# TheJacksonLaboratory/cnn_autoencoder

Hardware: AMD Instinct MI355X
Metric: tiles/sec, compress+decompress round trip of 1024x1024x3 histology tiles (higher is better)
Workload: dtype f32 (f16x3 split MFMA: 3 f16 MFMAs per product, fp32 accumulate)

## Files before the change

cnn_autoencoder_amd/csrc/cae_api.hip:

```cpp
#include "cae_hip.h"
#include "cae_internal.hpp"
#include "cae_kernels.hpp"
#include "cae_kernels_f16.hpp"
#include "cae_launch.hpp"
#include "cae_pack.hpp"

#include <algorithm>
#include <cmath>
#include <cstdio>
#include <cstdlib>
#include <cstring>
#include <string>

namespace cae {

thread_local std::string g_last_error;
thread_local int64_t g_last_ticket = 0;
thread_local int g_force_fp32 = 0;

int fail(int code, const char *fmt, ...) {
    char buf[512];
    va_list ap;
    va_start(ap, fmt);
    vsnprintf(buf, sizeof buf, fmt, ap);
    va_end(ap);
    g_last_error = buf;
    return code;
}

void dev_free(void *p) { (void)hipFree(p); }

int DevBuf::alloc(size_t n) {
    reset();
    HIP_TRY(hipMalloc(&p, n));
    bytes = n;
    return CAE_OK;
}

int DevBuf::upload(const void *src, size_t n) {
    CAE_TRY(alloc(n));
    HIP_TRY(hipMemcpy(p, src, n, hipMemcpyHostToDevice));
    return CAE_OK;
}

int Model::ensure_ws(int which, size_t bytes) {
    DevBuf &b = ws[which];
    if (b.bytes >= bytes) return CAE_OK;
    if (b) {
        HIP_TRY(hipDeviceSynchronize());
        b.reset();
    }
    return b.alloc((bytes + (1u << 20)) & ~(size_t)((1u << 20) - 1));
}

int Model::order_stream(void *stream) {
    if (last_stream_set && last_stream != stream) {
        if (!order_event) HIP_TRY(hipEventCreateWithFlags((hipEvent_t *)&order_event, hipEventDisableTiming));
        HIP_TRY(hipEventRecord((hipEvent_t)order_event, (hipStream_t)last_stream));
        HIP_TRY(hipStreamWaitEvent((hipStream_t)stream, (hipEvent_t)order_event, 0));
    }
    last_stream = stream;
    last_stream_set = true;
    return CAE_OK;
}

int Model::ensure_device() {
    if (!zero) {
        CAE_TRY(zero.alloc(1024));
        HIP_TRY(hipMemset(zero.p, 0, 1024));
    }
    if (medians_dirty && ent.channels > 0) {
        CAE_TRY(medians_dev.upload(ent.medians));
        medians_dirty = false;
    }
    if (density_dirty && !density.empty()) {
        CAE_TRY(density_dev.upload(density));
        density_dirty = false;
    }
    if (!flags) {
        HIP_TRY(hipHostMalloc((void **)&flags, kFlagSlots * sizeof(int), hipHostMallocMapped));
        memset(flags, 0, kFlagSlots * sizeof(int));
        HIP_TRY(hipHostGetDevicePointer((void **)&flags_dev, flags, 0));
    }
    return CAE_OK;
}

int *Model::next_flag(int64_t *ticket) {
    *ticket = ++flag_seq;
    const int slot = (int)(*ticket % kFlagSlots);
    *(volatile int *)(flags + slot) = 0;
    g_last_ticket = *ticket;
    return flags_dev + slot;
}

bool Model::f16_usable() const {
    if (precision != 1 || g_force_fp32) return false;
    for (auto *tr : {&enc, &dec})
        for (auto &l : *tr)
            if (l.set && l.f16_bad) return false;
    return true;
}

Model::~Model() {
    if (order_event) (void)hipEventDestroy((hipEvent_t)order_event);
    if (flags) (void)hipHostFree(flags);
}

struct ProfScope {
    Model *m;
    int track;
    hipStream_t st;
    std::vector<std::pair<void *, void *>> ev;
    hipEvent_t cur = nullptr;
    ProfScope(Model *m_, int track_, hipStream_t st_) : m(m_), track(track_), st(st_) {}
    void begin() {
        if (!m->profiling) return;
        hipEvent_t a;
        if (hipEventCreate(&a) != hipSuccess) return;
        (void)hipEventRecord(a, st);
        cur = a;
    }
    void end() {
        if (!m->profiling || !cur) return;
        hipEvent_t b;
        if (hipEventCreate(&b) != hipSuccess) return;
        (void)hipEventRecord(b, st);
        ev.emplace_back((void *)cur, (void *)b);
        cur = nullptr;
    }
    ~ProfScope() {
        if (m->profiling && !ev.empty()) m->prof[track].push_back(std::move(ev));
    }
};

static unsigned ew_grid(size_t total) {
    size_t b = (total + 255) / 256;
    return (unsigned)std::min<size_t>(std::max<size_t>(b, 1), 256 * 8 * 4);
}

static int layer_of(Model *m, int track, int index, Layer *&l) {
    if (track != CAE_ANALYSIS && track != CAE_SYNTHESIS) return fail(CAE_ERR_ARG, "bad track %d", track);
    if (index < 0 || index >= m->L) return fail(CAE_ERR_ARG, "layer index %d out of range", index);
    l = &(track == CAE_ANALYSIS ? m->enc : m->dec)[index];
    return CAE_OK;
}

static int upload_channels(DevBuf &d, const float *v, int c, int ct, float fill) {
    if (!v) {
        d.reset();
        return CAE_OK;
    }
    CAE_TRY(d.upload(pad_channels(v, c, ct, fill)));
    if ((uintptr_t)d.p % 16 != 0 || d.bytes != (size_t)ct * 32 * sizeof(float))
        return fail(CAE_ERR_HIP, "per-channel vector: device buffer %p (%zu bytes) is not a 16-byte aligned run of %d floats",
                    d.p, d.bytes, ct * 32);
    return CAE_OK;
}

static LayerArgs layer_args(const Model *m, const float *in, int in_planes, void *out, int n, int h, int w, int oh, int ow,
                            int ct, int cout, int outfmt, int act, int *flag) {
    LayerArgs a{};
    a.in = in;
    a.out = out;
    a.zero = m->zero.get<float>();
    a.medians = m->zero.get<float>();
    a.flag = flag;
    a.N = n;
    a.H = h;
    a.W = w;
    a.OH = oh;
    a.OW = ow;
    a.in_planes = in_planes;
    a.out_planes = ct * 4;
    a.cout = cout;
    a.outfmt = outfmt;
    a.act = act;
    return a;
}

}

using namespace cae;

template <int R>
static void launch_likelihood(Model *m, const float *y, int n, int hw, float *yhat, float *lik, double *part,
                              hipStream_t st) {
    hipLaunchKernelGGL(likelihood_kernel<R>, dim3(m->c_bn, n), dim3(256), 0, st, y, m->medians_dev.get<float>(),
                       m->density_dev.get<float>(), m->density_per_channel, m->density_k, m->density_bound,
                       m->likelihood_plain, m->c_bn, hw, yhat, lik, part);
}

static int set_stage(Model *m, int track, Layer &l, int stage, const float *w, const float *bias, const float *beta,
                     const float *gamma, int act, int add_residual, int post_act) {
    const int ctin = round_ct(l.cin);
    if (ctin < 0) return fail(CAE_ERR_UNSUPPORTED, "more than 192 channels not supported");
    if ((int)l.stages.size() <= stage) l.stages.resize(stage + 1);
    Layer::Stage &sg = l.stages[stage];
    const bool tr = track == CAE_SYNTHESIS;
    CAE_TRY(sg.wp.upload(pack_weights(w, tr, l.cin, l.cin, m->ks, ctin, tr)));
    CAE_TRY(upload_channels(sg.bias, bias, l.cin, ctin, 0.0f));
    sg.gdn = beta != nullptr;
    if (sg.gdn) {
        CAE_TRY(upload_channels(sg.beta, beta, l.cin, ctin, 1.0f));
        CAE_TRY(sg.gp.upload(pack_gamma(gamma, l.cin, ctin)));
    }
    sg.act = act;
    sg.add_res = add_residual != 0;
    sg.post_act = post_act;
    if (m->precision == 1) {
        if (!fits_f16(w, (size_t)l.cin * l.cin * m->ks * m->ks)) l.f16_bad = true;
        CAE_TRY(sg.wp16.upload(pack_weights_f16(w, tr, l.cin, l.cin, m->ks, ctin, tr)));
        if (sg.gdn) {
            if (!fits_f16(gamma, (size_t)l.cin * l.cin)) l.f16_bad = true;
            CAE_TRY(sg.gp16.upload(pack_gamma_f16(gamma, l.cin, ctin)));
        }
    }
    if (track == CAE_ANALYSIS) {
        l.wp_edge.reset();
        l.wp_edge16.reset();
    }
    return CAE_OK;
}

static int pick_slot(int a, int b) {
    for (int k = 1; k <= 3; ++k)
        if (k != a && k != b) return k;
    return 1;
}

static bool stages_need_fp32(const Layer &l) {
    if (round_ct(l.cin) <= 4) return false;
    for (const Layer::Stage &sg : l.stages)
        if (sg.gdn || sg.add_res || sg.post_act) return true;
    return false;
}

static int run_stages(Model *m, const Layer &l, bool synthesis, int n, int ch, int cw, const float *&cur, int &cur_idx,
                      int &cur_planes, hipStream_t st, bool f16 = false, int *flag = nullptr) {
    if (f16 && stages_need_fp32(l)) {
        const int tmp = pick_slot(cur_idx, cur_idx);
        const size_t rows = (size_t)n * cur_planes * ch;
        if (synthesis)
            hipLaunchKernelGGL(c8s_to_c8_kernel<true>, dim3(ew_grid(rows * cw)), dim3(256), 0, st, (const char *)cur,
                               (float *)m->ws[tmp].p, rows, cw);
        else
            hipLaunchKernelGGL(c8s_to_c8_kernel<false>, dim3(ew_grid(rows * cw)), dim3(256), 0, st, (const char *)cur,
                               (float *)m->ws[tmp].p, rows, cw);
        HIP_TRY(hipGetLastError());
        cur = (const float *)m->ws[tmp].p;
        cur_idx = tmp;
        int rc = run_stages(m, l, synthesis, n, ch, cw, cur, cur_idx, cur_planes, st, false, nullptr);
        if (rc) return rc;
        const int back = pick_slot(cur_idx, cur_idx);
        const size_t orows = (size_t)n * cur_planes * ch;
        if (synthesis)
            hipLaunchKernelGGL(c8_to_c8s_kernel<true>, dim3(ew_grid(orows * cw)), dim3(256), 0, st, cur, (char *)m->ws[back].p,
                               orows, cw, flag);
        else
            hipLaunchKernelGGL(c8_to_c8s_kernel<false>, dim3(ew_grid(orows * cw)), dim3(256), 0, st, cur, (char *)m->ws[back].p,
                               orows, cw, flag);
        HIP_TRY(hipGetLastError());
        cur = (const float *)m->ws[back].p;
        cur_idx = back;
        return CAE_OK;
    }
    const float *unit_in = cur;
    const int unit_idx = cur_idx, unit_planes = cur_planes;
    for (const Layer::Stage &sg : l.stages) {
        const int ctin = round_ct(l.cin);
        const int out_idx = pick_slot(unit_idx, cur_idx);
        LayerArgs b = layer_args(m, cur, cur_planes, m->ws[out_idx].p, n, ch, cw, ch, cw, ctin, l.cin, OUT_C8, sg.act,
                                 f16 ? flag : nullptr);
        b.bias = sg.bias.get<float>();
        b.beta = sg.beta.get<float>();
        b.res = sg.add_res ? unit_in : nullptr;
        b.res_planes = unit_planes;
        b.post_act = sg.post_act;
        int rc;
        if (f16) {
            if (!sg.wp16 || (sg.gdn && !sg.gp16)) return fail(CAE_ERR_ARG, "stage uploaded before precision 1 was selected");
            b.wp = sg.wp16.get<float>();
            b.gp = sg.gp16.get<float>();
            rc = launch_conv_s1_f16(m->ks, ctin, synthesis, sg.gdn, l.cin, b, st);
        } else {
            b.wp = sg.wp.get<float>();
            b.gp = sg.gp.get<float>();
            rc = launch_conv_s1(m->ks, ctin, synthesis, sg.gdn, l.cin, b, st);
        }
        if (rc) return rc;
        cur = (const float *)b.out;
        cur_idx = out_idx;
        cur_planes = ctin * 4;
    }
    return CAE_OK;
}

static int launch_color(Model *m, const Layer &l, bool f16, const float *in, int in_planes, int n, int h, int w, float *out,
                        int *flag, hipStream_t st) {
    const int ct = round_ct(l.color_cout);
    LayerArgs c = layer_args(m, in, in_planes, out, n, h, w, h, w, ct, l.color_cout, OUT_NCHW, 0, f16 ? flag : nullptr);
    c.bias = l.color_bias.get<float>();
    if (f16) {
        c.wp = l.color_wp16.get<float>();
        return launch_color_f16(m->ks, l.cout, c, st);
    }
    c.wp = l.color_wp.get<float>();
    return launch_conv_s1(m->ks, ct, false, false, l.cout, c, st);
}

extern "C" {

int cae_version(void) { return 1; }
const char *cae_last_error(void) { return g_last_error.c_str(); }
void cae_free(void *p) { free(p); }

int cae_model_create(int channels_org, int channels_net, int channels_bn, int compression_level, int kernel_size,
                     cae_model_t **out) {
    if (!out) return fail(CAE_ERR_ARG, "out is NULL");
    if (channels_org < 1 || channels_net < 1 || channels_bn < 1 || compression_level < 1)
        return fail(CAE_ERR_ARG, "bad model dimensions");
    if (kernel_size != 3 && kernel_size != 5)
        return fail(CAE_ERR_UNSUPPORTED, "kernel_size %d not supported (3 or 5)", kernel_size);
    Model *m = new Model();
    m->c_org = channels_org;
    m->c_net = channels_net;
    m->c_bn = channels_bn;
    m->L = compression_level;
    m->ks = kernel_size;
    m->enc.resize(m->L);
    m->dec.resize(m->L);
// ... 417 lines not shown
        for (int i = 0; i < nrun; ++i) {
            if (!m->dec[i].stages.empty())
                maxact = std::max(maxact, (size_t)n * round_ct(m->dec[i].cin) * 4 * ch * row_bytes(cw));
            ch *= 2;
            cw *= 2;
            if (i + 1 < m->L) maxact = std::max(maxact, (size_t)n * m->dec[i].ct * 4 * ch * row_bytes(cw));
        }
    }
    bool need_third_slot = false;
    for (int i = 0; i < nrun; ++i)
        need_third_slot |= m->dec[i].stages.size() > 1 || (f16 && stages_need_fp32(m->dec[i]));
    if (scale > 0 && !m->dec[stop].color_w4 && fmt == CAE_FMT_U8_HWC) {
        maxact = std::max(maxact, (size_t)n * m->dec[stop].color_cout * (lh << nrun) * (lw << nrun) * sizeof(float));
    }
    if ((rc = m->ensure_ws(0, in_bytes))) return rc;
    if (maxact && ((rc = m->ensure_ws(1, maxact)) || (rc = m->ensure_ws(2, maxact)))) return rc;
    if (maxact && need_third_slot && (rc = m->ensure_ws(3, maxact))) return rc;

    ProfScope prof(m, CAE_SYNTHESIS, st);
    prof.begin();
    const size_t tot = (size_t)n * p0 * lh * lw;
    if (f16)
        hipLaunchKernelGGL(nchw_to_c8s_kernel<true>, dim3(ew_grid(tot)), dim3(256), 0, st, latents, (char *)m->ws[0].p, n,
                           m->c_bn, lh, lw, p0, flag, symbols, m->medians_dev.get<float>());
    else
        hipLaunchKernelGGL(nchw_to_c8_kernel, dim3(ew_grid(tot)), dim3(256), 0, st, latents, (float *)m->ws[0].p, n,
                           m->c_bn, lh * lw, p0, symbols, m->medians_dev.get<float>());
    HIP_TRY(hipGetLastError());
    prof.end();

    bool use_pmap = false;
    if (f16 && scale == 0 && m->L >= 2 && m->ks == 3 && getenv("CAE_NO_PMAP") == nullptr) {
        const Layer &lp = m->dec[m->L - 2], &ll = m->dec[m->L - 1];
        use_pmap = ll.wp_pmap16 && !ll.gdn && ll.stages.empty() && lp.stages.empty() && lp.ct <= 4 && lp.cout == ll.cin &&
                   !(bridges && bridges[m->L - 2]) && !(colors && colors[m->L - 2]);
    }
    if (use_pmap) maxact = std::max(maxact, (size_t)n * (lh << (m->L - 1)) * (lw << (m->L - 1)) * 128);
    if (use_pmap && ((rc = m->ensure_ws(1, maxact)) || (rc = m->ensure_ws(2, maxact)))) return rc;

    const float *cur = (const float *)m->ws[0].p;
    int cur_planes = p0, ch = lh, cw = lw;
    int cur_idx = 0;
    for (int i = 0; i < nrun; ++i) {
        const Layer &l = m->dec[i];
        const bool last = i == m->L - 1;
        if (use_pmap && last) {
            prof.begin();
            const int gtx = (cw + 15) / 16, gty = (ch + 15) / 16;
            hipLaunchKernelGGL(pmap_gather_kernel, dim3((unsigned)((size_t)n * gtx * gty)), dim3(256), 0, st, cur,
                               l.bias.get<float>(), out, n, ch, cw, l.cout, fmt == CAE_FMT_U8_HWC ? OUT_U8HWC : OUT_NCHW, gtx,
                               gty);
            HIP_TRY(hipGetLastError());
            prof.end();
            break;
        }
        if (!l.stages.empty() && (rc = run_stages(m, l, true, n, ch, cw, cur, cur_idx, cur_planes, st, f16, flag))) return rc;
        const int out_idx = pick_slot(cur_idx, cur_idx);
        LayerArgs a = layer_args(m, cur, cur_planes, last ? out : m->ws[out_idx].p, n, ch, cw, 2 * ch, 2 * cw, l.ct, l.cout,
                                 last ? (fmt == CAE_FMT_U8_HWC ? OUT_U8HWC : OUT_NCHW) : OUT_C8, l.act, flag);
        a.wp = l.wp.get<float>();
        a.bias = l.bias.get<float>();
        a.gp = l.gp.get<float>();
        a.beta = l.beta.get<float>();
        if (use_pmap && i == m->L - 2) {
            a.outfmt = OUT_PMAP;
            a.pm = m->dec[m->L - 1].wp_pmap16.p;
        }
        prof.begin();
        if (f16) {
            a.gp = l.gp16.get<float>();
            if (last && l.wp_edge16 && last_f16_fits(m->ks, l.cin)) {
                a.wp = l.wp_edge16.get<float>();
                if ((rc = launch_last_f16(m->ks, l.cin, a, st))) return rc;
            } else {
                if (l.act && l.ct > 4)
                    return fail(CAE_ERR_UNSUPPORTED, "f16x3: LeakyReLU / ReLU synthesis layers wider than 128 channels run "
                                                     "on the fp32 path: set precision 0");
                a.wp = l.wp16.get<float>();
                if ((rc = launch_deconv_f16(m->ks, l.ct, l.gdn, l.cin, a, st))) return rc;
            }
        } else if (last && l.wp_edge) {
            a.wp = l.wp_edge.get<float>();
            if ((rc = launch_last(m->ks, l.cin, a, st))) return rc;
        } else {
            if ((rc = launch_deconv(m->ks, l.ct, l.gdn, l.cin, a, st))) return rc;
        }
        prof.end();
        if (!last && colors && colors[i]) {
            if (!l.color_wp) return fail(CAE_ERR_ARG, "colour layer %d not set", i);
            if (f16 && !l.color_wp16)
                return fail(CAE_ERR_UNSUPPORTED, "f16x3: colour layers to more than 32 channels run on the fp32 path: set precision 0");
            if ((rc = launch_color(m, l, f16, (const float *)a.out, l.ct * 4, n, a.OH, a.OW, colors[i], flag, st))) return rc;
        }
        if (!last && bridges && bridges[i]) {
            const size_t t2 = (size_t)n * l.cout * a.OH * a.OW;
            if (f16)
                hipLaunchKernelGGL(c8s_to_nchw_kernel<true>, dim3(ew_grid(t2)), dim3(256), 0, st, (const char *)a.out,
                                   bridges[i], n, l.cout, a.OH, a.OW, l.ct * 4);
            else
                hipLaunchKernelGGL(c8_to_nchw_kernel, dim3(ew_grid(t2)), dim3(256), 0, st, (const float *)a.out,
                                   bridges[i], n, l.cout, a.OH * a.OW, l.ct * 4);
            HIP_TRY(hipGetLastError());
        }
        cur = (const float *)a.out;
        cur_planes = l.ct * 4;
        ch = a.OH;
        cw = a.OW;
        cur_idx = out_idx;
    }
    if (scale > 0) {
        const Layer &l = m->dec[stop];
        const int ofmt = fmt == CAE_FMT_U8_HWC ? OUT_U8HWC : OUT_NCHW;
        prof.begin();
        if (l.color_w4) {
            if ((rc = launch_color_small(m->ks, f16, cur, cur_planes, l.cout, l.color_w4.get<float>(),
                                         l.color_bias.get<float>(), n, ch, cw, l.color_cout, out, ofmt, flag, st)))
                return rc;
        } else {
            float *img = ofmt == OUT_NCHW ? (float *)out : (float *)m->ws[pick_slot(cur_idx, cur_idx)].p;
            if ((rc = launch_color(m, l, f16, cur, cur_planes, n, ch, cw, img, flag, st))) return rc;
            if (ofmt == OUT_U8HWC && (rc = launch_nchw_to_u8hwc(img, out, n, l.color_cout, (size_t)ch * cw, st))) return rc;
        }
        prof.end();
    }
    return CAE_OK;
}

int cae_gdn_forward(cae_model_t *mm, int track, int index, const float *x, int n, int h, int w, float *y, void *stream) {
    Model *m = reinterpret_cast<Model *>(mm);
    if (!m || !x || !y) return fail(CAE_ERR_ARG, "NULL argument");
    Layer *lp;
    CAE_TRY(layer_of(m, track, index, lp));
    if (n < 1 || h < 1 || w < 1) return fail(CAE_ERR_ARG, "bad tensor shape");
    hipStream_t st = (hipStream_t)stream;
    std::lock_guard<std::mutex> lk(m->mu);
    const Layer &l = *lp;
    if (!l.set || !l.gdn) return fail(CAE_ERR_ARG, "layer has no GDN");
    const int planes = l.ct * 4;
    int rc;
    if ((rc = m->ensure_device()) || (rc = m->order_stream(stream))) return rc;
    if ((rc = m->ensure_ws(0, (size_t)n * planes * h * w * 32))) return rc;
    const size_t tot = (size_t)n * planes * h * w;
    hipLaunchKernelGGL(nchw_to_c8_kernel, dim3(ew_grid(tot)), dim3(256), 0, st, x, (float *)m->ws[0].p, n, l.cout, h * w,
                       planes);
    HIP_TRY(hipGetLastError());
    LayerArgs a = layer_args(m, (const float *)m->ws[0].p, planes, y, n, h, w, h, w, l.ct, l.cout, OUT_NCHW, 0, nullptr);
    a.gp = l.gp.get<float>();
    a.beta = l.beta.get<float>();
    return launch_gdn(l.ct, track == CAE_SYNTHESIS, a, st);
}

int cae_tile_sse(const uint8_t *a, const uint8_t *b, int n, size_t elems, double *sse, void *stream) {
    if (!a || !b || !sse) return fail(CAE_ERR_ARG, "NULL argument");
    if (n < 1 || n > 65535 || elems < 1) return fail(CAE_ERR_ARG, "bad shape");
    hipStream_t st = (hipStream_t)stream;
    unsigned long long *acc = reinterpret_cast<unsigned long long *>(sse);
    HIP_TRY(hipMemsetAsync(acc, 0, (size_t)n * 8, st));
    const unsigned bx = (unsigned)std::min<size_t>(std::max<size_t>(elems / 16 / 256, 1), 64);
    hipLaunchKernelGGL(tile_sse_kernel, dim3(bx, n), dim3(256), 0, st, a, b, elems, acc);
    HIP_TRY(hipGetLastError());
    hipLaunchKernelGGL(u64_to_f64_kernel, dim3((n + 255) / 256), dim3(256), 0, st, acc, sse, n);
    HIP_TRY(hipGetLastError());
    return CAE_OK;
}

int cae_tile_ssim(const uint8_t *a, const uint8_t *b, int n, int h, int w, int c, double *ssim, double *workspace,
                  size_t workspace_elems, void *stream) {
    if (!a || !b || !ssim || !workspace) return fail(CAE_ERR_ARG, "NULL argument");
    if (n < 1 || n > 65535 || c < 1) return fail(CAE_ERR_ARG, "bad shape");
    if (h < 7 || w < 7) return fail(CAE_ERR_ARG, "tiles must be at least 7x7 (the SSIM window)");
    const int oh = h - 6, ow = w - 6;
    const int bxr = (ow + 31) / 32, bpt = bxr * ((oh + 31) / 32);
    if (workspace_elems < (size_t)n * bpt)
        return fail(CAE_ERR_ARG, "workspace too small: %zu doubles needed", (size_t)n * bpt);
    hipStream_t st = (hipStream_t)stream;
    hipLaunchKernelGGL(tile_ssim_kernel, dim3(bpt, n), dim3(256), 0, st, a, b, h, w, c, bxr, bpt, workspace);
    HIP_TRY(hipGetLastError());
    hipLaunchKernelGGL(ssim_reduce_kernel, dim3(n), dim3(256), 0, st, workspace, bpt, (double)oh * ow * c, ssim);
    HIP_TRY(hipGetLastError());
    return CAE_OK;
}

int cae_tile_delta_e(const uint8_t *a, const uint8_t *b, int n, size_t pixels, double *delta, double *workspace,
                     size_t workspace_elems, void *stream) {
    if (!a || !b || !delta || !workspace) return fail(CAE_ERR_ARG, "NULL argument");
    if (n < 1 || n > 65535 || pixels < 1) return fail(CAE_ERR_ARG, "bad shape");
    const int bpt = (int)std::min<size_t>((pixels + 255) / 256, 128);
    if (workspace_elems < (size_t)n * bpt)
        return fail(CAE_ERR_ARG, "workspace too small: %zu doubles needed", (size_t)n * bpt);
    hipStream_t st = (hipStream_t)stream;
    hipLaunchKernelGGL(tile_delta_e_kernel, dim3(bpt, n), dim3(256), 0, st, a, b, pixels, bpt, workspace);
    HIP_TRY(hipGetLastError());
    hipLaunchKernelGGL(ssim_reduce_kernel, dim3(n), dim3(256), 0, st, workspace, bpt, (double)pixels, delta);
    HIP_TRY(hipGetLastError());
    return CAE_OK;
}

int cae_u8hwc_to_planes(const uint8_t *tiles, int n, int h, int w, int c, float *planes, void *stream) {
    if (!tiles || !planes) return fail(CAE_ERR_ARG, "NULL argument");
    if (n < 1 || h < 1 || w < 1 || c < 1) return fail(CAE_ERR_ARG, "bad shape");
    hipLaunchKernelGGL(u8hwc_to_planes_kernel, dim3(ew_grid((size_t)n * c * h * w)), dim3(256), 0, (hipStream_t)stream,
                       tiles, planes, n, h, w, c);
    HIP_TRY(hipGetLastError());
    return CAE_OK;
}

int cae_avgpool2(const float *in, int planes, int h, int w, float *out, void *stream) {
    if (!in || !out) return fail(CAE_ERR_ARG, "NULL argument");
    if (planes < 1 || h < 1 || w < 1) return fail(CAE_ERR_ARG, "bad shape");
    const int oh = (h + 2 * (h & 1) - 2) / 2 + 1, ow = (w + 2 * (w & 1) - 2) / 2 + 1;
    hipLaunchKernelGGL(avgpool2_kernel, dim3(ew_grid((size_t)planes * oh * ow)), dim3(256), 0, (hipStream_t)stream, in,
                       out, planes, h, w, oh, ow);
    HIP_TRY(hipGetLastError());
    return CAE_OK;
}

int cae_msssim_level(const float *x, const float *y, int planes, int h, int w, const float *window11, double *ssim_cs,
                     double *workspace, size_t workspace_elems, void *stream) {
    if (!x || !y || !window11 || !ssim_cs || !workspace) return fail(CAE_ERR_ARG, "NULL argument");
    if (planes < 1 || planes > 65535) return fail(CAE_ERR_ARG, "bad plane count");
    if (h < 11 || w < 11) return fail(CAE_ERR_ARG, "image smaller than the 11-tap window");
    const int oh = h - 10, ow = w - 10;
    const int bxr = (ow + 31) / 32, bpp = bxr * ((oh + 31) / 32);
    if (workspace_elems < (size_t)planes * bpp * 2)
        return fail(CAE_ERR_ARG, "workspace too small: %zu doubles needed", (size_t)planes * bpp * 2);
    hipStream_t st = (hipStream_t)stream;
    hipLaunchKernelGGL(msssim_level_kernel, dim3(bpp, planes), dim3(256), 0, st, x, y, h, w, bxr, bpp, window11, workspace);
    HIP_TRY(hipGetLastError());
    hipLaunchKernelGGL(msssim_reduce_kernel, dim3(planes), dim3(256), 0, st, workspace, bpp, (double)oh * ow, ssim_cs);
    HIP_TRY(hipGetLastError());
    return CAE_OK;
}

int cae_model_set_profiling(cae_model_t *mm, int enable) {
    Model *m = reinterpret_cast<Model *>(mm);
    if (!m) return fail(CAE_ERR_ARG, "NULL model");
    std::lock_guard<std::mutex> lk(m->mu);
    m->profiling = enable != 0;
    return CAE_OK;
}

int cae_model_get_profile(cae_model_t *mm, int track, double *ms, int n_slots, int *calls, int reset) {
    Model *m = reinterpret_cast<Model *>(mm);
    if (!m || !ms || n_slots < 1) return fail(CAE_ERR_ARG, "NULL argument");
    if (track != CAE_ANALYSIS && track != CAE_SYNTHESIS) return fail(CAE_ERR_ARG, "bad track %d", track);
    std::lock_guard<std::mutex> lk(m->mu);
    for (int i = 0; i < n_slots; ++i) ms[i] = 0.0;
    auto &calls_v = m->prof[track];
    for (auto &call : calls_v)
        for (size_t i = 0; i < call.size(); ++i) {
            HIP_TRY(hipEventSynchronize((hipEvent_t)call[i].second));
            float t = 0.f;
            HIP_TRY(hipEventElapsedTime(&t, (hipEvent_t)call[i].first, (hipEvent_t)call[i].second));
            if ((int)i < n_slots) ms[i] += t;
        }
    if (calls) *calls = (int)calls_v.size();
    if (reset) {
        for (auto &call : calls_v)
            for (auto &e : call) {
                (void)hipEventDestroy((hipEvent_t)e.first);
                (void)hipEventDestroy((hipEvent_t)e.second);
            }
        calls_v.clear();
    }
    return CAE_OK;
}

int cae_quantize(cae_model_t *mm, const float *latents, int n, int hw, int32_t *symbols, void *stream) {
    Model *m = reinterpret_cast<Model *>(mm);
    if (!m || !latents || !symbols) return fail(CAE_ERR_ARG, "NULL argument");
    if (m->ent.channels == 0) return fail(CAE_ERR_ARG, "entropy model not set");
    if (n < 1 || hw < 1) return fail(CAE_ERR_ARG, "bad shape");
    {
        std::lock_guard<std::mutex> lk(m->mu);
        int rc = m->ensure_device();
        if (rc) return rc;
    }
    const size_t total = (size_t)n * m->c_bn * hw;
    hipLaunchKernelGGL(quantize_kernel, dim3(ew_grid(total)), dim3(256), 0, (hipStream_t)stream, latents,
                       m->medians_dev.get<float>(), symbols, m->c_bn, hw, total);
    HIP_TRY(hipGetLastError());
    return CAE_OK;
}

int cae_model_set_density(cae_model_t *mm, int channels, int n_filters, const int *filters, const float *const *matrices,
                          const float *const *biases, const float *const *factors, float likelihood_bound) {
    Model *m = reinterpret_cast<Model *>(mm);
    if (!m || !filters || !matrices || !biases || !factors) return fail(CAE_ERR_ARG, "NULL argument");
    if (channels != m->c_bn) return fail(CAE_ERR_ARG, "density model has %d channels, model %d", channels, m->c_bn);
    if (n_filters < 1) return fail(CAE_ERR_UNSUPPORTED, "density network needs at least one hidden layer");
    int R = 0;
    for (int i = 0; i < n_filters; ++i) {
        if (filters[i] < 1) return fail(CAE_ERR_ARG, "filters[%d]=%d", i, filters[i]);
        R = std::max(R, filters[i]);
    }
    if (R > 8) return fail(CAE_ERR_UNSUPPORTED, "density filters wider than 8 are not supported (got %d)", R);
    for (int i = 0; i <= n_filters; ++i)
        if (!matrices[i] || !biases[i] || (i < n_filters && !factors[i])) return fail(CAE_ERR_ARG, "NULL parameter %d", i);
    const int K = n_filters;
    const int per = 3 * R + (K - 1) * (R * R + 2 * R) + R + 1;
    std::vector<float> packed((size_t)channels * per, 0.f);
    auto width = [&](int i) { return i == 0 ? 1 : (i == K + 1 ? 1 : filters[i - 1]); };
    for (int c = 0; c < channels; ++c) {
        float *o = packed.data() + (size_t)c * per;
        for (int i = 0; i <= K; ++i) {
            const int fin = width(i), fout = width(i + 1);
            const float *M = matrices[i] + (size_t)c * fout * fin;
            const float *b = biases[i] + (size_t)c * fout;
            const float *t = i < K ? factors[i] + (size_t)c * fout : nullptr;
            if (i == 0) {
                for (int j = 0; j < fout; ++j) { o[j] = M[j]; o[R + j] = b[j]; o[2 * R + j] = t[j]; }
                o += 3 * R;
            } else if (i < K) {
                for (int j = 0; j < fout; ++j) {
// ... 118 lines not shown
```

cnn_autoencoder_amd/csrc/cae_kernels.hpp:

```cpp
#pragma once
#include <hip/hip_runtime.h>
#include <stdint.h>
#include <type_traits>
#include <utility>

namespace cae {

typedef float f32x16 __attribute__((ext_vector_type(16)));
typedef float f32x4 __attribute__((ext_vector_type(4)));

enum OutFmt { OUT_C8 = 0, OUT_NCHW = 1, OUT_U8HWC = 2, OUT_SYM = 3, OUT_PMAP = 4 };

struct LayerArgs {
    const float *in;
    void *out;
    const float *wp;
    const float *bias;
    const float *gp;
    const float *beta;
    const float *zero;
    int N, H, W, OH, OW;
    int in_planes;
    int cci;
    int out_planes;
// ... 735 lines not shown
    for (size_t i = (size_t)blockIdx.x * blockDim.x + threadIdx.x; i < total; i += (size_t)gridDim.x * blockDim.x) {
        const size_t pix = i % HW;
        const size_t np = i / HW;
        const int plane = (int)(np % planes);
        const size_t n = np / planes;
        f32x4 lo, hi;
#pragma unroll
        for (int k = 0; k < 4; ++k) {
            const int c0 = plane * 8 + k, c1 = c0 + 4;
            if (sym) {
                lo[k] = c0 < C ? (float)sym[(n * C + c0) * HW + pix] + medians[c0] : 0.0f;
                hi[k] = c1 < C ? (float)sym[(n * C + c1) * HW + pix] + medians[c1] : 0.0f;
            } else {
                lo[k] = c0 < C ? in[(n * C + c0) * HW + pix] : 0.0f;
                hi[k] = c1 < C ? in[(n * C + c1) * HW + pix] : 0.0f;
            }
        }
        float *dst = out + i * 8;
        *(f32x4 *)dst = lo;
        *(f32x4 *)(dst + 4) = hi;
    }
}

static __global__ void c8_to_nchw_kernel(const float *in, float *out, int N, int C, int HW, int planes) {
    const size_t total = (size_t)N * C * HW;
    for (size_t i = (size_t)blockIdx.x * blockDim.x + threadIdx.x; i < total; i += (size_t)gridDim.x * blockDim.x) {
        const size_t pix = i % HW;
        const size_t nc = i / HW;
        const int c = (int)(nc % C);
        const size_t n = nc / C;
        out[i] = in[((n * planes + (c >> 3)) * HW + pix) * 8 + (c & 7)];
    }
}

static __global__ void quantize_kernel(const float *y, const float *medians, int32_t *sym, int C, int HW, size_t total) {
    for (size_t i = (size_t)blockIdx.x * blockDim.x + threadIdx.x; i < total; i += (size_t)gridDim.x * blockDim.x) {
        const int c = (int)((i / HW) % C);
        sym[i] = round_sym(y[i] - medians[c]);
    }
}

static __global__ void __launch_bounds__(1024)
quantize_export4_kernel(const float *y, const float *medians, int32_t *sym, int C, int HW4, size_t total4) {
    typedef int i32x4 __attribute__((ext_vector_type(4)));
    const size_t stride = (size_t)gridDim.x * blockDim.x;
    for (size_t i0 = (size_t)blockIdx.x * blockDim.x + threadIdx.x; i0 < total4; i0 += 4 * stride) {
        f32x4 v[4];
#pragma unroll
        for (int k = 0; k < 4; ++k) {
            const size_t i = i0 + k * stride;
            if (i < total4) v[k] = ((const f32x4 *)y)[i];
        }
#pragma unroll
        for (int k = 0; k < 4; ++k) {
            const size_t i = i0 + k * stride;
            if (i < total4) {
                const float med = medians[(i / HW4) % C];
                i32x4 q;
#pragma unroll
                for (int e = 0; e < 4; ++e) q[e] = round_sym(v[k][e] - med);
                ((i32x4 *)sym)[i] = q;
            }
        }
    }
}

static __global__ void dequantize_kernel(const int32_t *sym, const float *medians, float *y, int C, int HW, size_t total) {
    for (size_t i = (size_t)blockIdx.x * blockDim.x + threadIdx.x; i < total; i += (size_t)gridDim.x * blockDim.x) {
        const int c = (int)((i / HW) % C);
        y[i] = (float)sym[i] + medians[c];
    }
}

template <int R>
__device__ __forceinline__ float logits_cumulative(const float *__restrict__ p, int K, float x) {
    float v[R];
#pragma unroll
    for (int j = 0; j < R; ++j) {
        v[j] = p[j] * x + p[R + j];
        v[j] += p[2 * R + j] * tanhf(v[j]);
    }
    p += 3 * R;
    for (int i = 1; i < K; ++i) {
        float u[R];
#pragma unroll
        for (int j = 0; j < R; ++j) {
            float acc = 0.f;
#pragma unroll
            for (int k = 0; k < R; ++k) acc += p[j * R + k] * v[k];
            acc += p[R * R + j];
            u[j] = acc + p[R * R + R + j] * tanhf(acc);
        }
#pragma unroll
        for (int j = 0; j < R; ++j) v[j] = u[j];
        p += R * R + 2 * R;
    }
    float acc = 0.f;
#pragma unroll
    for (int k = 0; k < R; ++k) acc += p[k] * v[k];
    return acc + p[R];
}

__device__ __forceinline__ float sigmoidf(float x) { return 1.f / (1.f + expf(-x)); }

template <int R>
__global__ void __launch_bounds__(256)
likelihood_kernel(const float *__restrict__ y, const float *__restrict__ medians, const float *__restrict__ params,
                  int per_channel, int K, float bound, int plain, int C, int HW, float *__restrict__ yhat,
                  float *__restrict__ lik, double *__restrict__ bits_part) {
    const int c = blockIdx.x, n = blockIdx.y;
    const float *pc = params + (size_t)c * per_channel;
    const float med = medians[c];
    const size_t base = ((size_t)n * C + c) * HW;
    double bits = 0.0;
    for (int i = threadIdx.x; i < HW; i += 256) {
        const float q = rintf(y[base + i] - med) + med;
        const float lo = logits_cumulative<R>(pc, K, q - 0.5f);
        const float up = logits_cumulative<R>(pc, K, q + 0.5f);
        const float t = lo + up;
        const float sgn = t > 0.f ? -1.f : (t < 0.f ? 1.f : 0.f);
        float pr = plain ? sigmoidf(up) - sigmoidf(lo) : fabsf(sigmoidf(sgn * up) - sigmoidf(sgn * lo));
        pr = fmaxf(pr, bound);
        if (yhat) yhat[base + i] = q;
        if (lik) lik[base + i] = pr;
        bits -= (double)log2f(pr);
    }
    if (!bits_part) return;
    __shared__ double red[256];
    red[threadIdx.x] = bits;
    __syncthreads();
#pragma unroll
    for (int s = 128; s > 0; s >>= 1) {
        if ((int)threadIdx.x < s) red[threadIdx.x] += red[threadIdx.x + s];
        __syncthreads();
    }
    if (threadIdx.x == 0) bits_part[(size_t)n * C + c] = red[0];
}

static __global__ void bits_reduce_kernel(const double *part, int C, double *bits) {
    __shared__ double red[256];
    const int n = blockIdx.x;
    double a = 0.0;
    for (int c = threadIdx.x; c < C; c += 256) a += part[(size_t)n * C + c];
    red[threadIdx.x] = a;
    __syncthreads();
#pragma unroll
    for (int s = 128; s > 0; s >>= 1) {
        if ((int)threadIdx.x < s) red[threadIdx.x] += red[threadIdx.x + s];
        __syncthreads();
    }
    if (threadIdx.x == 0) bits[n] = red[0];
}

static __global__ void tile_sse_kernel(const uint8_t *a, const uint8_t *b, size_t elems, unsigned long long *out) {
    const int tile = blockIdx.y;
    const uint8_t *pa = a + (size_t)tile * elems, *pb = b + (size_t)tile * elems;
    unsigned long long acc = 0;
    const bool vec = ((((uintptr_t)pa) | ((uintptr_t)pb)) & 15) == 0;
    const size_t nvec = vec ? elems / 16 : 0;
    auto sq = [](const uint4 &va, const uint4 &vb) {
        const unsigned wa[4] = {va.x, va.y, va.z, va.w}, wb[4] = {vb.x, vb.y, vb.z, vb.w};
        unsigned same = 0, cross = 0;
#pragma unroll
        for (int k = 0; k < 4; ++k) {
            same = __builtin_amdgcn_udot4(wa[k], wa[k], same, false);
            same = __builtin_amdgcn_udot4(wb[k], wb[k], same, false);
            cross = __builtin_amdgcn_udot4(wa[k], wb[k], cross, false);
        }
        return same - 2u * cross;
    };
    const size_t stride = (size_t)gridDim.x * blockDim.x;
    size_t i = (size_t)blockIdx.x * blockDim.x + threadIdx.x;
    for (; i + stride < nvec; i += 2 * stride) {
        const uint4 va0 = ((const uint4 *)pa)[i], vb0 = ((const uint4 *)pb)[i];
        const uint4 va1 = ((const uint4 *)pa)[i + stride], vb1 = ((const uint4 *)pb)[i + stride];
        acc += sq(va0, vb0);
        acc += sq(va1, vb1);
    }
    if (i < nvec) acc += sq(((const uint4 *)pa)[i], ((const uint4 *)pb)[i]);
    if (vec) {
        if (blockIdx.x == 0)
            for (size_t i = nvec * 16 + threadIdx.x; i < elems; i += blockDim.x) {
                const int d = (int)pa[i] - (int)pb[i];
                acc += (unsigned)(d * d);
            }
    } else {
        for (size_t i = (size_t)blockIdx.x * blockDim.x + threadIdx.x; i < elems; i += (size_t)gridDim.x * blockDim.x) {
            const int d = (int)pa[i] - (int)pb[i];
            acc += (unsigned)(d * d);
        }
    }
#pragma unroll
    for (int off = 32; off > 0; off >>= 1) acc += __shfl_down(acc, off, 64);
    if ((threadIdx.x & 63) == 0) atomicAdd(out + tile, acc);
}

static __global__ void __launch_bounds__(256)
tile_ssim_kernel(const uint8_t *a, const uint8_t *b, int H, int W, int C, int bx_per_row, int blocks_per_tile,
                 double *part) {
    constexpr int T = 32, WIN = 7, IN = T + WIN - 1;
    __shared__ uint8_t sa[IN][IN + 2], sb[IN][IN + 2];
    __shared__ int hs[5][IN][T];
    __shared__ double red[256];
    const int tile = blockIdx.y, blk = blockIdx.x;
    const int by = blk / bx_per_row, bx = blk - by * bx_per_row;
    const int oy0 = by * T, ox0 = bx * T;
    const int OH = H - WIN + 1, OW = W - WIN + 1;
    const size_t base = (size_t)tile * H * W * C;
    const double C1 = (0.01 * 255.0) * (0.01 * 255.0), C2 = (0.03 * 255.0) * (0.03 * 255.0);
    const double cov_norm = 49.0 / 48.0;
    double acc = 0.0;
    for (int c = 0; c < C; ++c) {
        __syncthreads();
        for (int i = threadIdx.x; i < IN * IN; i += 256) {
            const int r = i / IN, x = i - r * IN;
            const int iy = oy0 + r, ix = ox0 + x;
            const bool ok = iy < H && ix < W;
            const size_t off = base + ((size_t)(ok ? iy : 0) * W + (ok ? ix : 0)) * C + c;
            sa[r][x] = ok ? a[off] : 0;
            sb[r][x] = ok ? b[off] : 0;
        }
        __syncthreads();
        for (int i = threadIdx.x; i < IN * T; i += 256) {
            const int r = i / T, x = i - r * T;
            int s0 = 0, s1 = 0, s2 = 0, s3 = 0, s4 = 0;
#pragma unroll
            for (int k = 0; k < WIN; ++k) {
                const int u = sa[r][x + k], v = sb[r][x + k];
                s0 += u;
                s1 += v;
                s2 += u * u;
                s3 += v * v;
                s4 += u * v;
            }
            hs[0][r][x] = s0;
            hs[1][r][x] = s1;
            hs[2][r][x] = s2;
            hs[3][r][x] = s3;
            hs[4][r][x] = s4;
        }
        __syncthreads();
        for (int i = threadIdx.x; i < T * T; i += 256) {
            const int y = i / T, x = i - y * T;
            if (oy0 + y < OH && ox0 + x < OW) {
                int s[5] = {0, 0, 0, 0, 0};
#pragma unroll
                for (int k = 0; k < WIN; ++k)
#pragma unroll
                    for (int q = 0; q < 5; ++q) s[q] += hs[q][y + k][x];
                {
#pragma clang fp contract(off)
                    const double ux = s[0] / 49.0, uy = s[1] / 49.0;
                    const double vx = cov_norm * (s[2] / 49.0 - ux * ux), vy = cov_norm * (s[3] / 49.0 - uy * uy);
                    const double vxy = cov_norm * (s[4] / 49.0 - ux * uy);
                    const double A1 = 2.0 * ux * uy + C1, A2 = 2.0 * vxy + C2;
                    const double B1 = ux * ux + uy * uy + C1, B2 = vx + vy + C2;
                    acc += (A1 * A2) / (B1 * B2);
                }
            }
        }
    }
    red[threadIdx.x] = acc;
    __syncthreads();
#pragma unroll
    for (int st = 128; st > 0; st >>= 1) {
        if ((int)threadIdx.x < st) red[threadIdx.x] += red[threadIdx.x + st];
        __syncthreads();
    }
    if (threadIdx.x == 0) part[(size_t)tile * blocks_per_tile + blk] = red[0];
}

static __global__ void ssim_reduce_kernel(const double *part, int blocks_per_tile, double samples, double *ssim) {
    __shared__ double red[256];
    const int tile = blockIdx.x;
    double v = 0.0;
    for (int i = threadIdx.x; i < blocks_per_tile; i += 256) v += part[(size_t)tile * blocks_per_tile + i];
    red[threadIdx.x] = v;
    __syncthreads();
#pragma unroll
    for (int st = 128; st > 0; st >>= 1) {
        if ((int)threadIdx.x < st) red[threadIdx.x] += red[threadIdx.x + st];
        __syncthreads();
    }
    if (threadIdx.x == 0) ssim[tile] = red[0] / samples;
}

__device__ __forceinline__ void rgb_to_lab(const double *lin, const uint8_t *px, double &L, double &A, double &B) {
#pragma clang fp contract(off)
    const double r = lin[px[0]], g = lin[px[1]], b = lin[px[2]];
    double x = (0.412453 * r + 0.357580 * g + 0.180423 * b) / 0.95047;
    double y = (0.212671 * r + 0.715160 * g + 0.072169 * b) / 1.0;
    double z = (0.019334 * r + 0.119193 * g + 0.950227 * b) / 1.08883;
    x = x > 0.008856 ? cbrt(x) : 7.787 * x + 16.0 / 116.0;
    y = y > 0.008856 ? cbrt(y) : 7.787 * y + 16.0 / 116.0;
    z = z > 0.008856 ? cbrt(z) : 7.787 * z + 16.0 / 116.0;
    L = 116.0 * y - 16.0;
    A = 500.0 * (x - y);
    B = 200.0 * (y - z);
}

static __global__ void __launch_bounds__(256)
tile_delta_e_kernel(const uint8_t *a, const uint8_t *b, size_t pixels, int blocks_per_tile, double *part) {
    __shared__ double lin[256];
    __shared__ double red[256];
    {
        const double v = threadIdx.x / 255.0;
        lin[threadIdx.x] = v > 0.04045 ? pow((v + 0.055) / 1.055, 2.4) : v / 12.92;
    }
    __syncthreads();
    const int tile = blockIdx.y;
    const uint8_t *pa = a + (size_t)tile * pixels * 3, *pb = b + (size_t)tile * pixels * 3;
    double acc = 0.0;
    for (size_t i = (size_t)blockIdx.x * 256 + threadIdx.x; i < pixels; i += (size_t)blocks_per_tile * 256) {
#pragma clang fp contract(off)
        double l0, a0, b0, l1, a1, b1;
        rgb_to_lab(lin, pa + 3 * i, l0, a0, b0);
        rgb_to_lab(lin, pb + 3 * i, l1, a1, b1);
        acc += sqrt((l0 - l1) * (l0 - l1) + (a0 - a1) * (a0 - a1) + (b0 - b1) * (b0 - b1));
    }
    red[threadIdx.x] = acc;
    __syncthreads();
#pragma unroll
    for (int st = 128; st > 0; st >>= 1) {
        if ((int)threadIdx.x < st) red[threadIdx.x] += red[threadIdx.x + st];
        __syncthreads();
    }
    if (threadIdx.x == 0) part[(size_t)tile * blocks_per_tile + blockIdx.x] = red[0];
}

static __global__ void u8hwc_to_planes_kernel(const uint8_t *in, float *out, int N, int H, int W, int C) {
    const size_t total = (size_t)N * C * H * W;
    for (size_t i = (size_t)blockIdx.x * blockDim.x + threadIdx.x; i < total; i += (size_t)gridDim.x * blockDim.x) {
        const size_t pix = i % ((size_t)H * W);
        const size_t nc = i / ((size_t)H * W);
        const int c = (int)(nc % C);
        const size_t n = nc / C;
        out[i] = (float)in[(n * H * W + pix) * C + c];
    }
}

static __global__ void avgpool2_kernel(const float *in, float *out, int planes, int H, int W, int OH, int OW) {
    const int ph = H & 1, pw = W & 1;
    const size_t total = (size_t)planes * OH * OW;
    for (size_t i = (size_t)blockIdx.x * blockDim.x + threadIdx.x; i < total; i += (size_t)gridDim.x * blockDim.x) {
        const int ox = (int)(i % OW), oy = (int)((i / OW) % OH);
        const size_t pl = i / ((size_t)OW * OH);
        float s = 0.f;
#pragma unroll
        for (int dy = 0; dy < 2; ++dy)
#pragma unroll
            for (int dx = 0; dx < 2; ++dx) {
                const int y = 2 * oy - ph + dy, x = 2 * ox - pw + dx;
                if (y >= 0 && y < H && x >= 0 && x < W) s += in[(pl * H + y) * W + x];
            }
        out[i] = s * 0.25f;
    }
}

static __global__ void __launch_bounds__(256)
msssim_level_kernel(const float *X, const float *Y, int H, int W, int bx_per_row, int bpp, const float *win, double *part) {
    constexpr int T = 32, WIN = 11, IN = T + WIN - 1;
    __shared__ float sx[IN][IN + 1], sy[IN][IN + 1];
    __shared__ float vs[5][T][IN + 1];
    __shared__ double red[2][256];
    __shared__ float g[WIN];
    if (threadIdx.x < WIN) g[threadIdx.x] = win[threadIdx.x];
    const int plane = blockIdx.y, blk = blockIdx.x;
    const int by = blk / bx_per_row, bx = blk - by * bx_per_row;
    const int oy0 = by * T, ox0 = bx * T;
    const int OH = H - WIN + 1, OW = W - WIN + 1;
    const float *px = X + (size_t)plane * H * W, *py = Y + (size_t)plane * H * W;
    for (int i = threadIdx.x; i < IN * IN; i += 256) {
        const int r = i / IN, x = i - r * IN;
        const int iy = oy0 + r, ix = ox0 + x;
        const bool ok = iy < H && ix < W;
        sx[r][x] = ok ? px[(size_t)iy * W + ix] : 0.f;
        sy[r][x] = ok ? py[(size_t)iy * W + ix] : 0.f;
    }
    __syncthreads();
    for (int i = threadIdx.x; i < T * IN; i += 256) {
        const int y = i / IN, x = i - y * IN;
        float a0 = 0.f, a1 = 0.f, a2 = 0.f, a3 = 0.f, a4 = 0.f;
#pragma unroll
        for (int k = 0; k < WIN; ++k) {
            const float u = sx[y + k][x], v = sy[y + k][x], w = g[k];
            a0 = fmaf(w, u, a0);
            a1 = fmaf(w, v, a1);
            a2 = fmaf(w, u * u, a2);
            a3 = fmaf(w, v * v, a3);
            a4 = fmaf(w, u * v, a4);
        }
        vs[0][y][x] = a0;
        vs[1][y][x] = a1;
        vs[2][y][x] = a2;
        vs[3][y][x] = a3;
        vs[4][y][x] = a4;
    }
    __syncthreads();
    const float C1 = (0.01f * 255.f) * (0.01f * 255.f), C2 = (0.03f * 255.f) * (0.03f * 255.f);
    double ssum = 0.0, csum = 0.0;
    for (int i = threadIdx.x; i < T * T; i += 256) {
        const int y = i / T, x = i - y * T;
        if (oy0 + y < OH && ox0 + x < OW) {
            float m[5] = {0.f, 0.f, 0.f, 0.f, 0.f};
#pragma unroll
            for (int k = 0; k < WIN; ++k)
#pragma unroll
                for (int q = 0; q < 5; ++q) m[q] = fmaf(g[k], vs[q][y][x + k], m[q]);
            {
#pragma clang fp contract(off)
                const float mu1 = m[0], mu2 = m[1];
                const float mu1_sq = mu1 * mu1, mu2_sq = mu2 * mu2, mu12 = mu1 * mu2;
                const float s1 = m[2] - mu1_sq, s2 = m[3] - mu2_sq, s12 = m[4] - mu12;
                const float cs = (2.f * s12 + C2) / (s1 + s2 + C2);
                const float ss = ((2.f * mu12 + C1) / (mu1_sq + mu2_sq + C1)) * cs;
                ssum += (double)ss;
                csum += (double)cs;
            }
        }
    }
    red[0][threadIdx.x] = ssum;
    red[1][threadIdx.x] = csum;
    __syncthreads();
#pragma unroll
    for (int st = 128; st > 0; st >>= 1) {
        if ((int)threadIdx.x < st) {
            red[0][threadIdx.x] += red[0][threadIdx.x + st];
            red[1][threadIdx.x] += red[1][threadIdx.x + st];
        }
        __syncthreads();
    }
    if (threadIdx.x == 0) {
        part[((size_t)plane * bpp + blk) * 2 + 0] = red[0][0];
        part[((size_t)plane * bpp + blk) * 2 + 1] = red[1][0];
    }
}

static __global__ void msssim_reduce_kernel(const double *part, int bpp, double samples, double *out) {
    __shared__ double red[2][256];
    const int plane = blockIdx.x;
    double a = 0.0, b = 0.0;
    for (int i = threadIdx.x; i < bpp; i += 256) {
        a += part[((size_t)plane * bpp + i) * 2 + 0];
        b += part[((size_t)plane * bpp + i) * 2 + 1];
    }
    red[0][threadIdx.x] = a;
    red[1][threadIdx.x] = b;
    __syncthreads();
#pragma unroll
    for (int st = 128; st > 0; st >>= 1) {
        if ((int)threadIdx.x < st) {
            red[0][threadIdx.x] += red[0][threadIdx.x + st];
            red[1][threadIdx.x] += red[1][threadIdx.x + st];
        }
        __syncthreads();
    }
    if (threadIdx.x == 0) {
        out[(size_t)plane * 2 + 0] = red[0][0] / samples;
        out[(size_t)plane * 2 + 1] = red[1][0] / samples;
    }
}

static __global__ void u64_to_f64_kernel(const unsigned long long *in, double *out, int n) {
    const int i = blockIdx.x * blockDim.x + threadIdx.x;
    if (i < n) out[i] = (double)in[i];
}

}
```

Baseline: 4021.

## Fuse tile SSE finalize into kernel via last-block atomic counter

Result: slower. 3885 (-3.4%).

```diff
diff --git a/cnn_autoencoder_amd/csrc/cae_api.hip b/cnn_autoencoder_amd/csrc/cae_api.hip
--- a/cnn_autoencoder_amd/csrc/cae_api.hip
+++ b/cnn_autoencoder_amd/csrc/cae_api.hip
@@ -176,6 +176,38 @@
     a.outfmt = outfmt;
     a.act = act;
     return a;
+}
+
+constexpr int kSseMaxTiles = 65535;
+struct SseCells {
+    unsigned long long *cells = nullptr;
+    hipStream_t last_stream = nullptr;
+    bool last_stream_set = false;
+    hipEvent_t order_event = nullptr;
+};
+static int sse_cells(hipStream_t st, unsigned long long *&cells) {
+    static std::map<int, SseCells> per_device;
+    int dev = 0;
+    HIP_TRY(hipGetDevice(&dev));
+    SseCells &c = per_device[dev];
+    if (!c.cells) {
+        void *p = nullptr;
+        HIP_TRY(hipMalloc(&p, (size_t)kSseMaxTiles * 8));
+        if (hipError_t e = hipMemset(p, 0, (size_t)kSseMaxTiles * 8); e != hipSuccess) {
+            (void)hipFree(p);
+            return fail(CAE_ERR_HIP, "hipMemset: %s", hipGetErrorString(e));
+        }
+        c.cells = static_cast<unsigned long long *>(p);
+    }
+    if (c.last_stream_set && c.last_stream != st) {
+        if (!c.order_event) HIP_TRY(hipEventCreateWithFlags(&c.order_event, hipEventDisableTiming));
+        HIP_TRY(hipEventRecord(c.order_event, c.last_stream));
+        HIP_TRY(hipStreamWaitEvent(st, c.order_event, 0));
+    }
+    c.last_stream = st;
+    c.last_stream_set = true;
+    cells = c.cells;
+    return CAE_OK;
 }
 
 }
@@ -899,14 +931,14 @@
 
 int cae_tile_sse(const uint8_t *a, const uint8_t *b, int n, size_t elems, double *sse, void *stream) {
     if (!a || !b || !sse) return fail(CAE_ERR_ARG, "NULL argument");
-    if (n < 1 || n > 65535 || elems < 1) return fail(CAE_ERR_ARG, "bad shape");
+    if (n < 1 || n > kSseMaxTiles || elems < 1 || elems > TILE_SSE_MAX_ELEMS)
+        return fail(CAE_ERR_ARG, "bad shape");
     hipStream_t st = (hipStream_t)stream;
-    unsigned long long *acc = reinterpret_cast<unsigned long long *>(sse);
-    HIP_TRY(hipMemsetAsync(acc, 0, (size_t)n * 8, st));
-    const unsigned bx = (unsigned)std::min<size_t>(std::max<size_t>(elems / 16 / 256, 1), 64);
-    hipLaunchKernelGGL(tile_sse_kernel, dim3(bx, n), dim3(256), 0, st, a, b, elems, acc);
-    HIP_TRY(hipGetLastError());
-    hipLaunchKernelGGL(u64_to_f64_kernel, dim3((n + 255) / 256), dim3(256), 0, st, acc, sse, n);
+    const unsigned bx = (unsigned)std::min<size_t>(std::max<size_t>(elems / 16 / 256, 1), TILE_SSE_MAX_BLOCKS);
+    std::lock_guard<std::mutex> lock(launch_mutex());
+    unsigned long long *cells = nullptr;
+    CAE_TRY(sse_cells(st, cells));
+    hipLaunchKernelGGL(tile_sse_kernel, dim3(bx, n), dim3(256), 0, st, a, b, elems, cells, sse);
     HIP_TRY(hipGetLastError());
     return CAE_OK;
 }
diff --git a/cnn_autoencoder_amd/csrc/cae_kernels.hpp b/cnn_autoencoder_amd/csrc/cae_kernels.hpp
--- a/cnn_autoencoder_amd/csrc/cae_kernels.hpp
+++ b/cnn_autoencoder_amd/csrc/cae_kernels.hpp
@@ -911,7 +911,11 @@
     if (threadIdx.x == 0) bits[n] = red[0];
 }
 
-static __global__ void tile_sse_kernel(const uint8_t *a, const uint8_t *b, size_t elems, unsigned long long *out) {
+constexpr int TILE_SSE_SUM_BITS = 56, TILE_SSE_MAX_BLOCKS = 64;
+constexpr size_t TILE_SSE_MAX_ELEMS = (size_t)1 << 40;
+constexpr int TILE_SSE_DEPTH = 4;
+static __global__ void __launch_bounds__(256)
+tile_sse_kernel(const uint8_t *a, const uint8_t *b, size_t elems, unsigned long long *cells, double *out) {
     const int tile = blockIdx.y;
     const uint8_t *pa = a + (size_t)tile * elems, *pb = b + (size_t)tile * elems;
     unsigned long long acc = 0;
@@ -930,13 +934,17 @@
     };
     const size_t stride = (size_t)gridDim.x * blockDim.x;
     size_t i = (size_t)blockIdx.x * blockDim.x + threadIdx.x;
-    for (; i + stride < nvec; i += 2 * stride) {
-        const uint4 va0 = ((const uint4 *)pa)[i], vb0 = ((const uint4 *)pb)[i];
-        const uint4 va1 = ((const uint4 *)pa)[i + stride], vb1 = ((const uint4 *)pb)[i + stride];
-        acc += sq(va0, vb0);
-        acc += sq(va1, vb1);
-    }
-    if (i < nvec) acc += sq(((const uint4 *)pa)[i], ((const uint4 *)pb)[i]);
+    for (; i + (TILE_SSE_DEPTH - 1) * stride < nvec; i += TILE_SSE_DEPTH * stride) {
+        uint4 va[TILE_SSE_DEPTH], vb[TILE_SSE_DEPTH];
+#pragma unroll
+        for (int k = 0; k < TILE_SSE_DEPTH; ++k) {
+            va[k] = ((const uint4 *)pa)[i + k * stride];
+            vb[k] = ((const uint4 *)pb)[i + k * stride];
+        }
+#pragma unroll
+        for (int k = 0; k < TILE_SSE_DEPTH; ++k) acc += sq(va[k], vb[k]);
+    }
+    for (; i < nvec; i += stride) acc += sq(((const uint4 *)pa)[i], ((const uint4 *)pb)[i]);
     if (vec) {
         if (blockIdx.x == 0)
             for (size_t i = nvec * 16 + threadIdx.x; i < elems; i += blockDim.x) {
@@ -951,7 +959,16 @@
     }
 #pragma unroll
     for (int off = 32; off > 0; off >>= 1) acc += __shfl_down(acc, off, 64);
-    if ((threadIdx.x & 63) == 0) atomicAdd(out + tile, acc);
+    __shared__ unsigned long long part[4];
+    if ((threadIdx.x & 63) == 0) part[threadIdx.x >> 6] = acc;
+    __syncthreads();
+    if (threadIdx.x != 0) return;
+    const unsigned long long mine = part[0] + part[1] + part[2] + part[3];
+    const unsigned long long before = __hip_atomic_fetch_add(cells + tile, mine + (1ull << TILE_SSE_SUM_BITS),
+                                                             __ATOMIC_RELAXED, __HIP_MEMORY_SCOPE_AGENT);
+    if ((before >> TILE_SSE_SUM_BITS) != gridDim.x - 1) return;
+    out[tile] = (double)((before & ((1ull << TILE_SSE_SUM_BITS) - 1)) + mine);
+    __hip_atomic_store(cells + tile, 0ull, __ATOMIC_RELAXED, __HIP_MEMORY_SCOPE_AGENT);
 }
 
 static __global__ void __launch_bounds__(256)
@@ -1220,9 +1237,4 @@
     }
 }
 
-static __global__ void u64_to_f64_kernel(const unsigned long long *in, double *out, int n) {
-    const int i = blockIdx.x * blockDim.x + threadIdx.x;
-    if (i < n) out[i] = (double)in[i];
-}
-
-}
+}
```
